# Corleno/Nonstationary_Multivariate_Gaussian_Process

Hardware: AMD Instinct MI355X
Metric: log-posterior evals/sec (N=2048, D=3 nonseparable GP) (higher is better)
Workload: dtype f64

## Files before the change

nonstationary_multivariate_gaussian_process_amd/csrc/nmgp_chol.hip:

```cpp
#include "nmgp_internal.h"
#include <cstring>

namespace nmgpk {

static inline int cdiv_c(long long a, long long b) { return (int)((a + b - 1) / b); }

typedef double v4d __attribute__((ext_vector_type(4)));

#define SY_BM 128
#define SY_BK 16
#define SY_LD (SY_BM + 16)
#define SY_SB 8

__device__ __forceinline__ int clamp_row_pair(int r, int rows) {
    int rc = r < rows - 1 ? r : rows - 2;
    return rc < 0 ? 0 : rc;
}

__device__ __forceinline__ double fast_recip(double p) {
    double x = __builtin_amdgcn_rcp(p);
    double e = fma(-p, x, 1.0);
    x = fma(x, e, x);
    e = fma(-p, x, 1.0);
    x = fma(x, e, x);
// ... 1542 lines not shown
#pragma unroll
        for (int kk = 0; kk < 4; ++kk) x0 = __builtin_amdgcn_mfma_f64_16x16x4f64(ai[kk], T[pp][kk], x0, 0, 0, 0);
        T[pp] = x0;
#pragma unroll
        for (int kk = 0; kk < 4; ++kk)
#pragma unroll
            for (int q = pp + 1; q < 4; ++q) {
                const double a = reinterpret_cast<const double*>(&ops[(q == 1 ? 0 : (q == 2 ? 1 : 3)) + pp][lane])[kk];
                T[q] = __builtin_amdgcn_mfma_f64_16x16x4f64(a, T[pp][kk], T[q], 0, 0, 0);
            }
    }
    if (v0) {
#pragma unroll
        for (int q = 0; q < 4; ++q)
#pragma unroll
            for (int r = 0; r < 4; ++r) A[(size_t)(16 * q + 4 * r + l4) * lda + row] = T[q][r];
    }
}

static void trsm_64(hipStream_t s, const double* L, int ldl, int nb, double* A, int lda, int rows, int batch,
                    long long bstride, bool precise) {
    if (rows <= 0) return;
    if (precise) {
        NMGP_LAUNCH(k_trsm_64, dim3(cdiv_c(rows, 64), batch), dim3(256), 0, s, L, ldl, nb, A, lda, rows, bstride);
    } else if (nb == 64) {
        NMGP_LAUNCH(k_trsm_64h<5>, dim3(cdiv_c(rows, 64), batch), dim3(256), 0, s, L, ldl, A, lda, rows, bstride);
    } else {
        const long long wgs = (long long)cdiv_c(rows, 128) * batch;
        const int reps = wgs >= 4096 ? 4 : (wgs >= 2048 ? 2 : 1);
        NMGP_LAUNCH(k_trsm_64m, dim3(cdiv_c(rows, 128 * reps), batch), dim3(256), 0, s, L, ldl, nb, A, lda, rows, bstride, reps);
    }
}

#define PS_XLD 66
#define PS_XPS_OFF 6656
#define PS_XS_OFF (PS_XPS_OFF + 64 * PS_XLD)
#define PS_SMEM_DOUBLES (PS_XS_OFF + 64 * PS_XLD)

template <int MODE, int OCC = 2>
__global__ __launch_bounds__(512, OCC) void k_panel_step(double* __restrict__ Ab, int lda, int ck, int has_prev_a,
                                                        int has_next_a,
                                                        int m_act, int pend, long long bstride, int* __restrict__ info,
                                                        int istride, int T, int u_mrows, int u_ncols, int u_kflags,
                                                        int u_tiles, int nbatch, int pre_a, int un_fresh, int u_tri,
                                                        long long* __restrict__ stamps) {
    const int has_prev = MODE == 0 ? has_prev_a : (MODE == 2 ? 1 : 0);
    const int has_next = MODE == 0 ? has_next_a : (MODE == 1 ? 1 : 0);
    const int pre = MODE == 0 ? pre_a : 0;
    constexpr int kOpsT = MODE == 1 ? 0 : 4096;
    constexpr int kXps = PS_XPS_OFF;
    constexpr int kXs = MODE == 1 ? 2560 : PS_XS_OFF;
    constexpr int kSmem = MODE == 1 ? 2560 + 64 * PS_XLD
                                    : (MODE == 2 ? 6656 : (PS_SMEM_DOUBLES > 4 * SY_BK * SY_LD ? PS_SMEM_DOUBLES : 4 * SY_BK * SY_LD));
    static_assert(MODE != 1 || sizeof(Potf2Lds) <= kSmem * sizeof(double), "the factorisation's LDS aliases the step's");
#define PS_STAMP(i)                                                              \
    do {                                                                         \
        if (stamps && blockIdx.x == 0 && threadIdx.x == 0) stamps[i] = (long long)wall_clock64(); \
    } while (0)
    PS_STAMP(0);
    __shared__ __attribute__((aligned(32))) double smem[kSmem];
    const int tid = threadIdx.x, lane = tid & 63, w = tid >> 6;
    const int l15 = lane & 15, l4 = lane >> 4;
    const int bx = (int)blockIdx.x / nbatch, by = (int)blockIdx.x - bx * nbatch;
    if (bx >= T) {
        if constexpr (MODE == 0) {
            const int t = bx - T + by * u_tiles;
            const double* Ap = Ab + (size_t)(ck - 64) * lda + (ck + 128);
            double* Cp = Ab + (size_t)(ck + 128) * lda + (ck + 128);
            syrk_tile_body<4, SY_BK>(Ap, lda, Cp, lda, u_mrows, u_ncols, 64, bstride, bstride, u_kflags, -u_tiles, nbatch, t, 0,
                                     0, smem, smem + 2 * SY_BK * SY_LD, u_tri, 0);
        }
        return;
    }
    double* A = Ab + (size_t)by * bstride;
    v4d* opsC = reinterpret_cast<v4d*>(smem);
    v4d* opsT = reinterpret_cast<v4d*>(smem + kOpsT);
    double* Xps = smem + (MODE == 0 ? kXps : 0);
    double* Xs = smem + (MODE == 2 ? 0 : kXs);
    const bool wg0 = bx == 0;
    const bool isC = wg0 && w < 4;
    const bool wg1 = pre && bx == 1;
    const bool isP = wg1 && w < 4;
    const int row = wg0 ? ck + 64 + 16 * w + l15 : ck + 128 + 128 * (bx - 1) + 16 * w + l15;
    const bool rv = row < m_act && !(wg0 && w >= 4);
    const int rowc = row < m_act ? row : (m_act - 1);
    const bool un_used = has_next && (has_prev || wg0);
    double oc[8], ot[5];
    v4d Xp[4], Tk[4], Un[4];
    const double* Lp = A + (size_t)(ck - 64) * lda;
    if (has_prev) {
#pragma unroll
        for (int j = 0; j < 8; ++j) {
            const int e = tid + 512 * j, q = e >> 10, sx = (e >> 6) & 15, l = e & 63;
            oc[j] = -Lp[(size_t)(4 * sx + (l >> 4)) * lda + ck + 16 * q + (l & 15)];
        }
    }
    {
        const double* L = A + (size_t)ck * lda + ck;
#pragma unroll
        for (int j = 0; j < 5; ++j) {
            const int idx = tid + 512 * j;
            const int blk = idx >> 8, kk = (idx >> 6) & 3, l = idx & 63;
            const int rr = l & 15, kc = 4 * kk + (l >> 4);
            double v;
            if (blk < 6) {
                const int q = blk == 0 ? 1 : (blk < 3 ? 2 : 3);
                const int pp = blk == 0 ? 0 : (blk < 3 ? blk - 1 : blk - 3);
                v = -L[(size_t)(16 * pp + kc) * lda + 16 * q + rr];
            } else {
                const int q = blk - 6;
                if (kc < rr) v = L[(size_t)(16 * q + rr) * lda + 16 * q + kc];
                else if (kc == rr) v = 1.0 / L[(size_t)(16 * q + rr) * lda + 16 * q + rr];
                else v = 0.0;
            }
            ot[j] = v;
        }
    }
    auto load_rows = [&]() {
#pragma unroll
        for (int q = 0; q < 4; ++q)
#pragma unroll
            for (int r = 0; r < 4; ++r) {
                const int c = 16 * q + 4 * r + l4;
                Tk[q][r] = rv ? A[(size_t)(ck + c) * lda + rowc] : 0.0;
                Xp[q][r] = (rv && has_prev) ? Lp[(size_t)c * lda + rowc] : 0.0;
                Un[q][r] = (rv && un_used && row < un_fresh) ? A[(size_t)(ck + 64 + c) * lda + rowc] : 0.0;
            }
    };
    if constexpr (MODE != 2) load_rows();
    if (has_prev) {
#pragma unroll
        for (int j = 0; j < 8; ++j) {
            const int e = tid + 512 * j, q = e >> 10, sx = (e >> 6) & 15, l = e & 63;
            smem[((q * 4 + (sx >> 2)) * 64 + l) * 4 + (sx & 3)] = oc[j];
        }
        if (isP) {
#pragma unroll
            for (int q = 0; q < 4; ++q)
#pragma unroll
                for (int r = 0; r < 4; ++r) Xps[(16 * w + l15) * PS_XLD + 16 * q + 4 * r + l4] = Xp[q][r];
        }
    }
#pragma unroll
    for (int j = 0; j < 5; ++j) {
        const int idx = tid + 512 * j;
        const int blk = idx >> 8, kk = (idx >> 6) & 3, l = idx & 63;
        smem[kOpsT + (blk * 64 + l) * 4 + kk] = ot[j];
    }
    if constexpr (MODE == 2) load_rows();
    __syncthreads();
    PS_STAMP(1);
    if (has_prev && has_next && !wg0) {
#pragma unroll
        for (int j = 0; j < 8; ++j) {
            const int e = tid + 512 * j, q = e >> 10, sx = (e >> 6) & 15, l = e & 63;
            oc[j] = -Lp[(size_t)(4 * sx + (l >> 4)) * lda + ck + 64 + 16 * q + (l & 15)];
        }
    }
    if (has_prev && (!wg0 || isC)) {
#pragma unroll
        for (int sg = 0; sg < 4; ++sg)
#pragma unroll
            for (int kk = 0; kk < 4; ++kk)
#pragma unroll
                for (int q = 0; q < 4; ++q) {
                    const double a = reinterpret_cast<const double*>(&opsC[(q * 4 + sg) * 64 + lane])[kk];
                    Tk[q] = __builtin_amdgcn_mfma_f64_16x16x4f64(a, Xp[sg][kk], Tk[q], 0, 0, 0);
                }
    }
    PS_STAMP(2);
#pragma unroll
    for (int pp = 0; pp < 4; ++pp) {
        const v4d ai = opsT[(6 + pp) * 64 + lane];
        v4d x0 = {0.0, 0.0, 0.0, 0.0};
#pragma unroll
        for (int kk = 0; kk < 4; ++kk) x0 = __builtin_amdgcn_mfma_f64_16x16x4f64(ai[kk], Tk[pp][kk], x0, 0, 0, 0);
        Tk[pp] = x0;
#pragma unroll
        for (int kk = 0; kk < 4; ++kk)
#pragma unroll
            for (int q = pp + 1; q < 4; ++q) {
                const double a = reinterpret_cast<const double*>(&opsT[((q == 1 ? 0 : (q == 2 ? 1 : 3)) + pp) * 64 + lane])[kk];
                Tk[q] = __builtin_amdgcn_mfma_f64_16x16x4f64(a, Tk[pp][kk], Tk[q], 0, 0, 0);
            }
    }
    if (rv) {
#pragma unroll
        for (int q = 0; q < 4; ++q)
#pragma unroll
            for (int r = 0; r < 4; ++r) A[(size_t)(ck + 16 * q + 4 * r + l4) * lda + row] = Tk[q][r];
    }
    PS_STAMP(3);
    if (!has_next) return;
    if (!wg0) {
        if (isP) {
#pragma unroll
            for (int q = 0; q < 4; ++q)
#pragma unroll
                for (int r = 0; r < 4; ++r) Xs[(16 * w + l15) * PS_XLD + 16 * q + 4 * r + l4] = Tk[q][r];
        }
        if (wg1 && !has_prev) __syncthreads();
        if (has_prev) {
            __syncthreads();
#pragma unroll
            for (int j = 0; j < 8; ++j) {
                const int e = tid + 512 * j, q = e >> 10, sx = (e >> 6) & 15, l = e & 63;
                smem[((q * 4 + (sx >> 2)) * 64 + l) * 4 + (sx & 3)] = oc[j];
            }
            __syncthreads();
#pragma unroll
            for (int sg = 0; sg < 4; ++sg)
#pragma unroll
                for (int kk = 0; kk < 4; ++kk)
#pragma unroll
                    for (int q = 0; q < 4; ++q) {
                        const double a = reinterpret_cast<const double*>(&opsC[(q * 4 + sg) * 64 + lane])[kk];
                        Un[q] = __builtin_amdgcn_mfma_f64_16x16x4f64(a, Xp[sg][kk], Un[q], 0, 0, 0);
                    }
        }
        if (rv && (has_prev || row >= un_fresh)) {
#pragma unroll
            for (int q = 0; q < 4; ++q)
#pragma unroll
                for (int r = 0; r < 4; ++r) A[(size_t)(ck + 64 + 16 * q + 4 * r + l4) * lda + row] = Un[q][r];
        }
        if (isP) {
#pragma unroll 1
            for (int q0 = 0; q0 < 4; q0 += 2) {
                v4d Vn[2];
#pragma unroll
                for (int qq = 0; qq < 2; ++qq)
#pragma unroll
                    for (int r = 0; r < 4; ++r) Vn[qq][r] = A[(size_t)(ck + 128 + 16 * (q0 + qq) + 4 * r + l4) * lda + rowc];
                if (has_prev) {
#pragma unroll
                    for (int sg = 0; sg < 4; ++sg)
#pragma unroll
                        for (int kk = 0; kk < 4; ++kk)
#pragma unroll
                            for (int qq = 0; qq < 2; ++qq) {
                                const double a = -Xps[(16 * (q0 + qq) + l15) * PS_XLD + 16 * sg + 4 * kk + l4];
                                const double b = Xps[(16 * w + l15) * PS_XLD + 16 * sg + 4 * kk + l4];
                                Vn[qq] = __builtin_amdgcn_mfma_f64_16x16x4f64(a, b, Vn[qq], 0, 0, 0);
                            }
                }
#pragma unroll
                for (int sg = 0; sg < 4; ++sg)
#pragma unroll
                    for (int kk = 0; kk < 4; ++kk)
#pragma unroll
                        for (int qq = 0; qq < 2; ++qq) {
                            const double a = -Xs[(16 * (q0 + qq) + l15) * PS_XLD + 16 * sg + 4 * kk + l4];
                            const double b = Xs[(16 * w + l15) * PS_XLD + 16 * sg + 4 * kk + l4];
                            Vn[qq] = __builtin_amdgcn_mfma_f64_16x16x4f64(a, b, Vn[qq], 0, 0, 0);
                        }
#pragma unroll
                for (int qq = 0; qq < 2; ++qq)
#pragma unroll
                    for (int r = 0; r < 4; ++r) A[(size_t)(ck + 128 + 16 * (q0 + qq) + 4 * r + l4) * lda + row] = Vn[qq][r];
            }
        }
        return;
    }
    if (isC) {
#pragma unroll
        for (int q = 0; q < 4; ++q)
#pragma unroll
            for (int r = 0; r < 4; ++r) Xs[(16 * w + l15) * PS_XLD + 16 * q + 4 * r + l4] = Tk[q][r];
    }
    PS_STAMP(4);
    __syncthreads();
    PS_STAMP(5);
    if (isC) {
#pragma unroll
        for (int sg = 0; sg < 4; ++sg)
#pragma unroll
            for (int kk = 0; kk < 4; ++kk)
#pragma unroll
                for (int q = 0; q < 4; ++q) {
                    const double a = -Xs[(16 * q + l15) * PS_XLD + 16 * sg + 4 * kk + l4];
                    Un[q] = __builtin_amdgcn_mfma_f64_16x16x4f64(a, Tk[sg][kk], Un[q], 0, 0, 0);
                }
    }
    Potf2Lds& P = *reinterpret_cast<Potf2Lds*>(smem);
    __syncthreads();
    if (isC) {
#pragma unroll
        for (int q = 0; q < 4; ++q)
#pragma unroll
            for (int r = 0; r < 4; ++r) {
                const int rr = 16 * w + l15, cc = 16 * q + 4 * r + l4;
                P.S[cc * PB_LD + rr] = (cc <= rr) ? Un[q][r] : 0.0;
            }
    }
    __syncthreads();
    PS_STAMP(6);
    potf2b_core_mfma(P, info + (size_t)by * istride, ck + 64);
    PS_STAMP(7);
    potf2b_store(A + (size_t)(ck + 64) * lda + (ck + 64), lda, 64, P, tid, 512);
    PS_STAMP(8);
#undef PS_STAMP
}

template <int NP, bool FACT, int OCC>
__global__ __launch_bounds__(512, OCC) void k_leaf_step(double* __restrict__ Ab, int lda, int ck, int m_act, long long bstride,
                                                       int* __restrict__ info, int istride, int T, int nbatch, int t_fresh0,
                                                       int t_fresh1) {
    constexpr int kOpsC = 2560;
    constexpr int kSmem = kOpsC + (FACT ? 64 * PS_XLD : 4096);
    static_assert(64 * PS_XLD >= 4096, "Xs aliases (and covers) the catch-up operands");
    static_assert(!FACT || sizeof(Potf2Lds) <= kSmem * sizeof(double), "the factorisation's LDS aliases the step's");
    static_assert(64 * NP <= 64 * NMGP_XTRI_SEED_BLOCKS, "the catch-up of a row of L^-T would read left of the seeded band");
    __shared__ __attribute__((aligned(32))) double smem[kSmem];
    const int tid = threadIdx.x, lane = tid & 63, w = tid >> 6;
    const int l15 = lane & 15, l4 = lane >> 4;
    const int bx = (int)blockIdx.x / nbatch, by = (int)blockIdx.x - bx * nbatch;
    double* A = Ab + (size_t)by * bstride;
    v4d* opsT = reinterpret_cast<v4d*>(smem);
    v4d* opsC = reinterpret_cast<v4d*>(smem + kOpsC);
    double* Xs = smem + kOpsC;
    const bool wg0 = bx == 0;
    const bool isC = wg0 && w < 4;
    const int row = wg0 ? ck + 64 + 16 * w + l15 : ck + 128 + 128 * (bx - 1) + 16 * w + l15;
    const bool rv = row < m_act && !(wg0 && w >= 4);
    const int rowc = row < m_act ? row : (m_act - 1);
    const bool tload = rv && !(row >= t_fresh0 && row < t_fresh1);
    const int wu = __builtin_amdgcn_readfirstlane(w);
    const unsigned vrow = (unsigned)(l4 * lda + rowc), vops = (unsigned)(l4 * lda + l15);
    auto colp = [&](int col) { return A + (size_t)col * lda; };
    double oc[8], ot[5];
    v4d Xp[4], Tk[4];
    auto load_ops = [&](int p) {
        const int cb = ck - 64 * (NP - p);
#pragma unroll
        for (int j = 0; j < 8; ++j) oc[j] = -(colp(cb + 4 * (wu + 8 * (j & 1))) + ck + 16 * (j >> 1))[vops];
    };
    auto store_ops = [&]() {
#pragma unroll
        for (int j = 0; j < 8; ++j) smem[kOpsC + (((j >> 1) * 4 + (j & 1) * 2 + (wu >> 2)) * 64 + lane) * 4 + (wu & 3)] = oc[j];
    };
    auto load_x = [&](int p) {
        const int cb = ck - 64 * (NP - p);
#pragma unroll
        for (int q = 0; q < 4; ++q) Xp[q] = v4d{0.0, 0.0, 0.0, 0.0};
        if (rv) {
#pragma unroll
            for (int q = 0; q < 4; ++q)
#pragma unroll
                for (int r = 0; r < 4; ++r) Xp[q][r] = colp(cb + 16 * q + 4 * r)[vrow];
        }
    };
    load_ops(0);
    {
        const double* L = A + (size_t)ck * lda + ck;
#pragma unroll
        for (int j = 0; j < 5; ++j) {
            const int idx = tid + 512 * j;
            const int blk = idx >> 8, kk = (idx >> 6) & 3, l = idx & 63;
            const int rr = l & 15, kc = 4 * kk + (l >> 4);
            double v;
            if (blk < 6) {
                const int q = blk == 0 ? 1 : (blk < 3 ? 2 : 3);
                const int pp = blk == 0 ? 0 : (blk < 3 ? blk - 1 : blk - 3);
                v = -L[(size_t)(16 * pp + kc) * lda + 16 * q + rr];
            } else {
                const int q = blk - 6;
                if (kc < rr) v = L[(size_t)(16 * q + rr) * lda + 16 * q + kc];
                else if (kc == rr) v = 1.0 / L[(size_t)(16 * q + rr) * lda + 16 * q + rr];
                else v = 0.0;
            }
            ot[j] = v;
        }
    }
    store_ops();
#pragma unroll
    for (int j = 0; j < 5; ++j) {
        const int idx = tid + 512 * j;
        const int blk = idx >> 8, kk = (idx >> 6) & 3, l = idx & 63;
        smem[(blk * 64 + l) * 4 + kk] = ot[j];
    }
#pragma unroll
    for (int q = 0; q < 4; ++q) Tk[q] = v4d{0.0, 0.0, 0.0, 0.0};
    if (tload) {
#pragma unroll
        for (int q = 0; q < 4; ++q)
#pragma unroll
            for (int r = 0; r < 4; ++r) Tk[q][r] = colp(ck + 16 * q + 4 * r)[vrow];
    }
    load_x(0);
    __syncthreads();
#pragma unroll
    for (int p = 0; p < NP; ++p) {
        if (!wg0 || isC) {
#pragma unroll
            for (int sg = 0; sg < 4; ++sg)
#pragma unroll
                for (int kk = 0; kk < 4; ++kk)
#pragma unroll
                    for (int q = 0; q < 4; ++q) {
                        const double a = reinterpret_cast<const double*>(&opsC[(q * 4 + sg) * 64 + lane])[kk];
                        Tk[q] = __builtin_amdgcn_mfma_f64_16x16x4f64(a, Xp[sg][kk], Tk[q], 0, 0, 0);
                    }
        }
        if (p + 1 < NP) {
            __syncthreads();
            load_ops(p + 1);
            if constexpr (OCC > 4) {
                store_ops();
                __builtin_amdgcn_sched_barrier(0);
                load_x(p + 1);
            } else {
                load_x(p + 1);
                store_ops();
            }
            __syncthreads();
        }
    }
#pragma unroll
    for (int pp = 0; pp < 4; ++pp) {
        const v4d ai = opsT[(6 + pp) * 64 + lane];
        v4d x0 = {0.0, 0.0, 0.0, 0.0};
#pragma unroll
        for (int kk = 0; kk < 4; ++kk) x0 = __builtin_amdgcn_mfma_f64_16x16x4f64(ai[kk], Tk[pp][kk], x0, 0, 0, 0);
        Tk[pp] = x0;
#pragma unroll
        for (int kk = 0; kk < 4; ++kk)
#pragma unroll
            for (int q = pp + 1; q < 4; ++q) {
                const double a = reinterpret_cast<const double*>(&opsT[((q == 1 ? 0 : (q == 2 ? 1 : 3)) + pp) * 64 + lane])[kk];
                Tk[q] = __builtin_amdgcn_mfma_f64_16x16x4f64(a, Tk[pp][kk], Tk[q], 0, 0, 0);
            }
    }
    if (rv) {
#pragma unroll
        for (int q = 0; q < 4; ++q)
#pragma unroll
            for (int r = 0; r < 4; ++r) colp(ck + 16 * q + 4 * r)[vrow] = Tk[q][r];
    }
    if constexpr (FACT) {
        if (!wg0) return;
        v4d Un[4];
        if (isC) {
#pragma unroll
            for (int q = 0; q < 4; ++q)
#pragma unroll
                for (int r = 0; r < 4; ++r) Un[q][r] = colp(ck + 64 + 16 * q + 4 * r)[vrow];
        }
#pragma unroll 1
        for (int p = 0; p < NP; ++p) {
            const int cb = ck - 64 * (NP - p);
#pragma unroll
            for (int j = 0; j < 8; ++j) oc[j] = colp(cb + wu + 8 * j)[ck + 64 + lane];
            __syncthreads();
#pragma unroll
            for (int j = 0; j < 8; ++j) Xs[lane * PS_XLD + wu + 8 * j] = oc[j];
            __syncthreads();
            if (isC) {
#pragma unroll
                for (int sg = 0; sg < 4; ++sg)
#pragma unroll
                    for (int kk = 0; kk < 4; ++kk) {
                        const double b = Xs[(16 * w + l15) * PS_XLD + 16 * sg + 4 * kk + l4];
#pragma unroll
                        for (int q = 0; q < 4; ++q) {
                            const double a = -Xs[(16 * q + l15) * PS_XLD + 16 * sg + 4 * kk + l4];
                            Un[q] = __builtin_amdgcn_mfma_f64_16x16x4f64(a, b, Un[q], 0, 0, 0);
                        }
                    }
            }
        }
        __syncthreads();
        if (isC) {
#pragma unroll
            for (int q = 0; q < 4; ++q)
#pragma unroll
                for (int r = 0; r < 4; ++r) Xs[(16 * w + l15) * PS_XLD + 16 * q + 4 * r + l4] = Tk[q][r];
        }
        __syncthreads();
        if (isC) {
#pragma unroll
            for (int sg = 0; sg < 4; ++sg)
#pragma unroll
                for (int kk = 0; kk < 4; ++kk)
#pragma unroll
                    for (int q = 0; q < 4; ++q) {
                        const double a = -Xs[(16 * q + l15) * PS_XLD + 16 * sg + 4 * kk + l4];
                        Un[q] = __builtin_amdgcn_mfma_f64_16x16x4f64(a, Tk[sg][kk], Un[q], 0, 0, 0);
                    }
        }
        Potf2Lds& P = *reinterpret_cast<Potf2Lds*>(smem);
        __syncthreads();
        if (isC) {
#pragma unroll
            for (int q = 0; q < 4; ++q)
#pragma unroll
                for (int r = 0; r < 4; ++r) {
                    const int rr = 16 * w + l15, cc = 16 * q + 4 * r + l4;
                    P.S[cc * PB_LD + rr] = (cc <= rr) ? Un[q][r] : 0.0;
                }
        }
        __syncthreads();
        potf2b_core_mfma(P, info + (size_t)by * istride, ck + 64);
        potf2b_store(A + (size_t)(ck + 64) * lda + (ck + 64), lda, 64, P, tid, 512);
    }
}

__global__ void k_set_row(double* __restrict__ A, int lda, int row, const double* __restrict__ v, int n,
                          long long bstride, long long vstride, int cps) {
    int j = blockIdx.x * blockDim.x + threadIdx.x;
    if (j < n) A[(size_t)blockIdx.y * bstride + (size_t)j * lda + row] = v[(size_t)(blockIdx.y / cps) * vstride + j];
}
void set_row(hipStream_t s, double* A, int lda, int row, const double* v, int n, int batch, long long bstride,
             long long vstride, int cps) {
    NMGP_LAUNCH(k_set_row, dim3(cdiv_c(n, 256), batch), dim3(256), 0, s, A, lda, row, v, n, bstride, vstride, cps < 1 ? 1 : cps);
}
__global__ void k_get_row(const double* __restrict__ A, int lda, int row, double* __restrict__ v, int n,
                          long long bstride, long long vstride) {
    int j = blockIdx.x * blockDim.x + threadIdx.x;
    if (j < n) v[(size_t)blockIdx.y * vstride + j] = A[(size_t)blockIdx.y * bstride + (size_t)j * lda + row];
}
void get_row(hipStream_t s, const double* A, int lda, int row, double* v, int n, int batch, long long bstride,
             long long vstride) {
    NMGP_LAUNCH(k_get_row, dim3(cdiv_c(n, 256), batch), dim3(256), 0, s, A, lda, row, v, n, bstride, vstride);
}

struct Factorisation {
    hipStream_t s, s2;
    double* A;
    int lda, n, extra, xtri;
    int* info;
    int batch;
    long long bs;
    int is;
    bool precise;
    const SyrkHook* hook;
    long long* stamps;
    bool block_done = false;

    double* at(int row, int col) const { return A + (size_t)col * lda + row; }
    int active_rows(int cend) const { return n + extra + (cend < xtri ? cend : xtri); }
    bool take_block_done() {
        const bool done = block_done;
        block_done = false;
        return done;
    }

    void update(hipStream_t st, int c0, int k, int c1, int ncols, int fuse_width) {
        const bool fuse = fuse_width >= 64 && !precise;
        const bool done = syrk_lower(st, at(c1, c0), lda, at(c1, c1), lda, active_rows(c0 + k) - c1, ncols, k, batch, bs, -1, 0,
                                     xtri > 0 ? n + extra - c1 : kNoTriRows, c0, fuse ? info : nullptr, is, c1, hook);
        if (fuse) block_done = done;
    }

    void block_solve(int c0, int w) {
        if (!take_block_done()) potf2_64(s, at(c0, c0), lda, w, info, c0, batch, bs, is, precise);
        trsm_64(s, at(c0, c0), lda, w, at(c0 + w, c0), lda, active_rows(c0 + w) - (c0 + w), batch, bs, precise);
    }

    void fused_steps(int c0, int w, bool leaf) {
        if (!take_block_done()) potf2_64(s, at(c0, c0), lda, 64, info, c0, batch, bs, is, precise);
        const int nk = w / 64;
        for (int k = 0; k < nk; ++k) {
            const int ck = c0 + 64 * k;
            const int m_act = active_rows(ck + 64);
            const int rows = m_act - (ck + 64);
            if (rows <= 0) continue;
            const int has_prev = k > 0, has_next = k + 1 < nk;
            const int T = 1 + (rows > 64 ? cdiv_c(rows - 64, 128) : 0);
            SyrkPlan pl;
            const int u_m = m_act - (ck + 128), u_n = c0 + w - (ck + 128);
            if (has_prev && u_m > 0 && u_n > 0) pl = syrk_plan(lda, lda, u_m, u_n, 64, 1, 0, true);
            const int pre = (ck + 192 <= c0 + w) ? 1 : 0;
            if (pre) pl.kflags |= 128;
            long long* st = stamps ? stamps + (size_t)(ck / 64) * 16 : nullptr;
            const int un_fresh = xtri > 0 ? n + extra + (has_prev ? ck - 64 : ck) : kNoTriRows;
            const int u_tri = xtri > 0 ? n + extra - 64 * NMGP_XTRI_SEED_BLOCKS : kNoTriRows;
            if (leaf && pl.tiles == 0 && !pre && nk == 2) {
                if (k == 0)
                    NMGP_LAUNCH((k_panel_step<1, 4>), dim3((unsigned)(T * batch)), dim3(512), 0, s, A, lda, ck, 0, 1, m_act, c0 + w, bs, info,
                                is, T, 0, 0, 0, 0, batch, 0, un_fresh, u_tri, st);
                else
                    NMGP_LAUNCH((k_panel_step<2, 6>), dim3((unsigned)(T * batch)), dim3(512), 0, s, A, lda, ck, 1, 0, m_act, c0 + w, bs, info,
                                is, T, 0, 0, 0, 0, batch, 0, un_fresh, u_tri, st);
            } else {
                NMGP_LAUNCH((k_panel_step<0, 2>), dim3((unsigned)((T + pl.tiles) * batch)), dim3(512), 0, s, A, lda, ck, has_prev, has_next, m_act,
                            c0 + w, bs, info, is, T, pl.mrows, u_n, pl.kflags, pl.tiles, batch, pre, un_fresh, u_tri, st);
            }
        }
    }

    void leaf256(int c0) {
        if (!take_block_done()) potf2_64(s, at(c0, c0), lda, 64, info, c0, batch, bs, is, precise);
        const int f0 = xtri > 0 ? n + extra + c0 : kNoTriRows;
        for (int k = 0; k < 4; ++k) {
            const int ck = c0 + 64 * k;
            const int m_act = active_rows(ck + 64);
            const int rows = m_act - (ck + 64);
            if (rows <= 0) continue;
            const int T = 1 + (rows > 64 ? cdiv_c(rows - 64, 128) : 0);
            const dim3 grid((unsigned)(T * batch));
            if (k == 0)
                NMGP_LAUNCH((k_panel_step<1, 4>), grid, dim3(512), 0, s, A, lda, ck, 0, 1, m_act, c0 + 128, bs, info, is, T, 0, 0, 0, 0, batch,
                            0, f0, xtri > 0 ? n + extra - 64 * NMGP_XTRI_SEED_BLOCKS : kNoTriRows,
                            stamps ? stamps + (size_t)(ck / 64) * 16 : nullptr);
            else if (k == 1)
                NMGP_LAUNCH((k_leaf_step<1, true, 4>), grid, dim3(512), 0, s, A, lda, ck, m_act, bs, info, is, T, batch, kNoTriRows,
                            kNoTriRows);
            else if (k == 2)
                NMGP_LAUNCH((k_leaf_step<2, true, 4>), grid, dim3(512), 0, s, A, lda, ck, m_act, bs, info, is, T, batch, f0,
                            xtri > 0 ? f0 + 128 : kNoTriRows);
            else
                NMGP_LAUNCH((k_leaf_step<3, false, 6>), grid, dim3(512), 0, s, A, lda, ck, m_act, bs, info, is, T, batch, f0,
                            xtri > 0 ? f0 + 192 : kNoTriRows);
        }
    }

    void panel_rl(int c0, int w) {
        for (int j0 = c0; j0 < c0 + w; j0 += 64) {
            const int jb = (c0 + w - j0 < 64) ? (c0 + w - j0) : 64;
            block_solve(j0, jb);
            update(s, j0, jb, j0 + jb, c0 + w - (j0 + jb), c0 + w - (j0 + jb));
        }
    }

    enum Leaf {
        kBlockSolve,
        kFusedSteps,
        kLeaf128
    };
    void panel_halving(int c0, int w, int base, Leaf leaf) {
        if (w <= base) {
            if (leaf == kBlockSolve || (leaf == kLeaf128 && w != 128)) block_solve(c0, w);
            else fused_steps(c0, w, leaf == kLeaf128);
            return;
        }
        if (leaf == kLeaf128 && w == 256) {
            leaf256(c0);
            return;
        }
        int h = ((w / 2 + 63) / 64) * 64;
        if (h >= w) h = ((w - 1) / 64) * 64;
        panel_halving(c0, h, base, leaf);
        update(s, c0, h, c0 + h, w - h, w - h);
        panel_halving(c0 + h, w - h, base, leaf);
    }

    void panel(int c0, int w) {
        const Switches& sw = switches();
        const bool mfma_ok = w > 0 && (w % 64 == 0) && (lda % 2 == 0) && !precise;
        const bool small = sw.fused_max_batch >= 0 ? batch <= sw.fused_max_batch : (long long)batch * n <= 73728;
        const int rec_min_batch = 4;
        if (mfma_ok && (sw.panel == Switches::kFused || (sw.panel == Switches::kAuto && small)))
            panel_halving(c0, w, fused_base(w), kFusedSteps);
        else if (mfma_ok && sw.panel == Switches::kAuto && batch >= rec_min_batch && w >= 128)
            panel_halving(c0, w, 128, kLeaf128);
        else if (sw.panel == Switches::kRl || (sw.panel != Switches::kRec && batch < rec_min_batch))
            panel_rl(c0, w);
        else
            panel_halving(c0, w, 64, kBlockSolve);
    }
    int fused_base(int w) const {
        if (switches().fused_base >= 64) return switches().fused_base;
        if (w > 256 && (batch >= 16 || (xtri > 0 && batch >= 5))) return 256;
        return w;
    }

    void run(int nb1, hipEvent_t* ev) {
        const bool la = (s2 != nullptr && ev != nullptr && n > 2 * nb1 && batch <= switches().la_max_batch && !precise);
        if (!la) {
            for (int c0 = 0; c0 < n; c0 += nb1) {
                const int w1 = (n - c0 < nb1) ? (n - c0) : nb1;
                const int c1 = c0 + w1;
                panel(c0, w1);
                update(s, c0, w1, c1, n - c1, n - c1 < nb1 ? n - c1 : nb1);
            }
            return;
        }
        hipEventRecord(ev[0], s);
        hipStreamWaitEvent(s2, ev[0], 0);
        int k = 0;
        bool prevB = false;
        for (int c0 = 0; c0 < n; c0 += nb1, ++k) {
            const int w1 = (n - c0 < nb1) ? (n - c0) : nb1;
            const int c1 = c0 + w1;
            const int w1n = (c1 < n) ? ((n - c1 < nb1) ? (n - c1) : nb1) : 0;
            const int c2 = c1 + w1n;
            hipEvent_t evPanel = ev[1 + 2 * k], evB = ev[2 + 2 * k];
            panel(c0, w1);
            if (c1 >= n) break;
            if (prevB) hipStreamWaitEvent(s, ev[2 + 2 * (k - 1)], 0);
            update(s, c0, w1, c1, w1n, w1n);
            hipEventRecord(evPanel, s);
            prevB = false;
            if (c2 < n) {
                hipStreamWaitEvent(s2, evPanel, 0);
                update(s2, c0, w1, c2, n - c2, 0);
                hipEventRecord(evB, s2);
                prevB = true;
            }
        }
        if (prevB) hipStreamWaitEvent(s, ev[2 + 2 * (k - 1)], 0);
    }
};

void potrf_lower(hipStream_t s, hipStream_t s2, hipEvent_t* ev, double* A, int lda, int n, int extra, int xtri,
                 int nb1, int* info, int batch, long long bstride, int istride, const SyrkHook* hook, int precise) {
    if (nb1 <= 0)
        nb1 = (batch >= 16 && n >= 4096) ? 2048
              : (((batch >= 4 && n >= 4096) || (batch >= 32 && n >= 2048)) && (long long)batch * n > 73728) ? 1024 : 512;
    const int nsteps = (n + 63) / 64;
    Factorisation f{s, s2, A, lda, n, extra, xtri, info, batch, bstride, istride, precise != 0, hook, g_step_stamps.begin(s, nsteps)};
    f.run(nb1, ev);
    g_step_stamps.dump(s, nsteps);
}

static_assert(SY_BM + 2 * SY_BK - 2 <= 64 * NMGP_XTRI_SEED_BLOCKS, "update tiles of L^-T rows would read left of the seeded band");
static_assert(NMGP_XTRI_SEED_BLOCKS == 3, "k_panel_step (u_tri) and k_xtri_seed's grid (4 column blocks per row block) assume three seeded blocks");
__global__ __launch_bounds__(256) void k_xtri_seed(double* __restrict__ A, int lda, int row0, int n, int pad,
                                                    long long bstride) {
    A += (size_t)blockIdx.z * bstride;
    const int lane = threadIdx.x & 63, w = threadIdx.x >> 6;
    if (blockIdx.x == gridDim.x - 1) {
        for (int c = blockIdx.y * 256 + threadIdx.x; c < n; c += 256 * gridDim.y)
            for (int q = 0; q < pad; ++q) A[(size_t)c * lda + row0 + q] = 0.0;
        return;
    }
    const int b = blockIdx.x;
    const int r = 64 * b + lane;
    const int cb = b - NMGP_XTRI_SEED_BLOCKS + (int)blockIdx.y;
    if (cb < 0 || r >= n) return;
#pragma unroll 4
    for (int k = 0; k < 16; ++k) {
        const int c = 64 * cb + w + 4 * k;
        if (c < n) A[(size_t)c * lda + row0 + pad + r] = (r == c) ? 1.0 : 0.0;
    }
}
void identity_rows(hipStream_t s, double* A, int lda, int row0, int n, int pad, int batch, long long bstride) {
    NMGP_LAUNCH(k_xtri_seed, dim3(cdiv_c(n, 64) + 1, NMGP_XTRI_SEED_BLOCKS + 1, batch), dim3(256), 0, s, A, lda, row0, n, pad, bstride);
}

}
```

Before: 1734.

## Pipeline next-panel loads under MFMA in leaf step via buffer loads

```diff
diff --git a/nonstationary_multivariate_gaussian_process_amd/csrc/nmgp_chol.hip b/nonstationary_multivariate_gaussian_process_amd/csrc/nmgp_chol.hip
--- a/nonstationary_multivariate_gaussian_process_amd/csrc/nmgp_chol.hip
+++ b/nonstationary_multivariate_gaussian_process_amd/csrc/nmgp_chol.hip
@@ -1868,8 +1868,8 @@
 #undef PS_STAMP
 }
 
-template <int NP, bool FACT, int OCC>
-__global__ __launch_bounds__(512, OCC) void k_leaf_step(double* __restrict__ Ab, int lda, int ck, int m_act, long long bstride,
+template <int NP, bool FACT>
+__global__ __launch_bounds__(512, 4) void k_leaf_step(double* __restrict__ Ab, int lda, int ck, int m_act, long long bstride,
                                                        int* __restrict__ info, int istride, int T, int nbatch, int t_fresh0,
                                                        int t_fresh1) {
     constexpr int kOpsC = 2560;
@@ -1899,23 +1899,21 @@
     auto load_ops = [&](int p) {
         const int cb = ck - 64 * (NP - p);
 #pragma unroll
-        for (int j = 0; j < 8; ++j) oc[j] = -(colp(cb + 4 * (wu + 8 * (j & 1))) + ck + 16 * (j >> 1))[vops];
+        for (int j = 0; j < 8; ++j) oc[j] = (colp(cb + 4 * (wu + 8 * (j & 1))) + ck + 16 * (j >> 1))[vops];
     };
     auto store_ops = [&]() {
-#pragma unroll
-        for (int j = 0; j < 8; ++j) smem[kOpsC + (((j >> 1) * 4 + (j & 1) * 2 + (wu >> 2)) * 64 + lane) * 4 + (wu & 3)] = oc[j];
+        __builtin_amdgcn_sched_barrier(0);
+#pragma unroll
+        for (int j = 0; j < 8; ++j) smem[kOpsC + (((j >> 1) * 4 + (j & 1) * 2 + (wu >> 2)) * 64 + lane) * 4 + (wu & 3)] = -oc[j];
     };
-    auto load_x = [&](int p) {
-        const int cb = ck - 64 * (NP - p);
-#pragma unroll
-        for (int q = 0; q < 4; ++q) Xp[q] = v4d{0.0, 0.0, 0.0, 0.0};
-        if (rv) {
-#pragma unroll
-            for (int q = 0; q < 4; ++q)
-#pragma unroll
-                for (int r = 0; r < 4; ++r) Xp[q][r] = colp(cb + 16 * q + 4 * r)[vrow];
-        }
+    auto row_block = [&](int cb) { return __builtin_amdgcn_make_buffer_rsrc(colp(cb), (short)0, 0x7fffffff, 0x00020000); };
+    auto load_group = [&](v4d& dst, __amdgpu_buffer_rsrc_t blk, int g, unsigned voff) {
+#pragma unroll
+        for (int r = 0; r < 4; ++r)
+            dst[r] = __builtin_bit_cast(double, __builtin_amdgcn_raw_buffer_load_b64(blk, (int)voff, (16 * g + 4 * r) * lda * 8, 0));
     };
+    const unsigned kMasked = 0x80000000u;
+    const unsigned vxoff = rv ? vrow * 8u : kMasked, vtoff = tload ? vrow * 8u : kMasked;
     load_ops(0);
     {
         const double* L = A + (size_t)ck * lda + ck;
@@ -1924,42 +1922,41 @@
             const int idx = tid + 512 * j;
             const int blk = idx >> 8, kk = (idx >> 6) & 3, l = idx & 63;
             const int rr = l & 15, kc = 4 * kk + (l >> 4);
-            double v;
-            if (blk < 6) {
+            if (j < 3) {
                 const int q = blk == 0 ? 1 : (blk < 3 ? 2 : 3);
                 const int pp = blk == 0 ? 0 : (blk < 3 ? blk - 1 : blk - 3);
-                v = -L[(size_t)(16 * pp + kc) * lda + 16 * q + rr];
+                ot[j] = L[(size_t)(16 * pp + kc) * lda + 16 * q + rr];
             } else {
                 const int q = blk - 6;
-                if (kc < rr) v = L[(size_t)(16 * q + rr) * lda + 16 * q + kc];
-                else if (kc == rr) v = 1.0 / L[(size_t)(16 * q + rr) * lda + 16 * q + rr];
-                else v = 0.0;
-            }
-            ot[j] = v;
-        }
+                ot[j] = L[(size_t)(16 * q + rr) * lda + 16 * q + (kc < rr ? kc : rr)];
+            }
+        }
+    }
+    {
+        const __amdgpu_buffer_rsrc_t own = row_block(ck), x0 = row_block(ck - 64 * NP);
+#pragma unroll
+        for (int q = 0; q < 4; ++q) load_group(Tk[q], own, q, vtoff);
+#pragma unroll
+        for (int q = 0; q < 4; ++q) load_group(Xp[q], x0, q, vxoff);
     }
     store_ops();
 #pragma unroll
     for (int j = 0; j < 5; ++j) {
         const int idx = tid + 512 * j;
         const int blk = idx >> 8, kk = (idx >> 6) & 3, l = idx & 63;
-        smem[(blk * 64 + l) * 4 + kk] = ot[j];
-    }
-#pragma unroll
-    for (int q = 0; q < 4; ++q) Tk[q] = v4d{0.0, 0.0, 0.0, 0.0};
-    if (tload) {
-#pragma unroll
-        for (int q = 0; q < 4; ++q)
-#pragma unroll
-            for (int r = 0; r < 4; ++r) Tk[q][r] = colp(ck + 16 * q + 4 * r)[vrow];
-    }
-    load_x(0);
+        const int rr = l & 15, kc = 4 * kk + (l >> 4);
+        const double v = j < 3 ? -ot[j] : (kc < rr ? ot[j] : (kc == rr ? 1.0 / ot[j] : 0.0));
+        smem[(blk * 64 + l) * 4 + kk] = v;
+    }
     __syncthreads();
 #pragma unroll
     for (int p = 0; p < NP; ++p) {
-        if (!wg0 || isC) {
-#pragma unroll
-            for (int sg = 0; sg < 4; ++sg)
+        const bool more = p + 1 < NP;
+        if (more) load_ops(p + 1);
+        const __amdgpu_buffer_rsrc_t xnext = row_block(ck - 64 * (NP - p - 1));
+#pragma unroll
+        for (int sg = 0; sg < 4; ++sg) {
+            if (!wg0 || isC) {
 #pragma unroll
                 for (int kk = 0; kk < 4; ++kk)
 #pragma unroll
@@ -1967,18 +1964,12 @@
                         const double a = reinterpret_cast<const double*>(&opsC[(q * 4 + sg) * 64 + lane])[kk];
                         Tk[q] = __builtin_amdgcn_mfma_f64_16x16x4f64(a, Xp[sg][kk], Tk[q], 0, 0, 0);
                     }
-        }
-        if (p + 1 < NP) {
+            }
+            if (more) load_group(Xp[sg], xnext, sg, vxoff);
+        }
+        if (more) {
             __syncthreads();
-            load_ops(p + 1);
-            if constexpr (OCC > 4) {
-                store_ops();
-                __builtin_amdgcn_sched_barrier(0);
-                load_x(p + 1);
-            } else {
-                load_x(p + 1);
-                store_ops();
-            }
+            store_ops();
             __syncthreads();
         }
     }
@@ -2170,13 +2161,13 @@
                             0, f0, xtri > 0 ? n + extra - 64 * NMGP_XTRI_SEED_BLOCKS : kNoTriRows,
                             stamps ? stamps + (size_t)(ck / 64) * 16 : nullptr);
             else if (k == 1)
-                NMGP_LAUNCH((k_leaf_step<1, true, 4>), grid, dim3(512), 0, s, A, lda, ck, m_act, bs, info, is, T, batch, kNoTriRows,
+                NMGP_LAUNCH((k_leaf_step<1, true>), grid, dim3(512), 0, s, A, lda, ck, m_act, bs, info, is, T, batch, kNoTriRows,
                             kNoTriRows);
             else if (k == 2)
-                NMGP_LAUNCH((k_leaf_step<2, true, 4>), grid, dim3(512), 0, s, A, lda, ck, m_act, bs, info, is, T, batch, f0,
+                NMGP_LAUNCH((k_leaf_step<2, true>), grid, dim3(512), 0, s, A, lda, ck, m_act, bs, info, is, T, batch, f0,
                             xtri > 0 ? f0 + 128 : kNoTriRows);
             else
-                NMGP_LAUNCH((k_leaf_step<3, false, 6>), grid, dim3(512), 0, s, A, lda, ck, m_act, bs, info, is, T, batch, f0,
+                NMGP_LAUNCH((k_leaf_step<3, false>), grid, dim3(512), 0, s, A, lda, ck, m_act, bs, info, is, T, batch, f0,
                             xtri > 0 ? f0 + 192 : kNoTriRows);
         }
     }
```

After: 1770, median of 6. +2.1%, better.
